# tpfeifle/pointcloud-segmentation-attention

Measured on AMD Instinct MI355X. Metric: 8192-pt clouds/sec through SA+FP layers, 1/2/4/8 MI355X; HBM GB/s vs peak, higher is better.
Workload: dtype f32

## Files before the change

pointcloud-segmentation-attention_amd/csrc/interp.hip:

```cpp
#include <algorithm>
#include <type_traits>

#include "grid.h"

namespace pn2 {
namespace {

constexpr int kNNBlock = 256;
constexpr int kNNGroup = 4;
constexpr int kNNRows = kNNBlock / kNNGroup;
constexpr int kNNTile = 2048;

struct Best3 {
  float d1, d2, d3;
  int i1, i2, i3;
};

PN2_DEV void best3_init(Best3& b) {
  b.d1 = b.d2 = b.d3 = __builtin_inff();
  b.i1 = b.i2 = b.i3 = 0;
}

PN2_DEV void best3_insert(Best3& b, float d, int k) {
  const bool c1 = d < b.d1, c2 = d < b.d2, c3 = d < b.d3;
// ... 86 lines not shown
  best3_merge_xor(best, 2);
}

__global__ __launch_bounds__(kNNBlock) void three_nn_kernel(const float* __restrict__ xyz1,
                                                            const float* __restrict__ xyz2, int n,
                                                            int m, float* __restrict__ dist,
                                                            int32_t* __restrict__ idx) {
  __shared__ float4 sk[kNNTile];
  const int b = blockIdx.y;
  const int j = blockIdx.x * kNNRows + threadIdx.x / kNNGroup;
  const bool valid = j < n;
  const float* U = xyz1 + ((size_t)b * n + (valid ? j : 0)) * 3;
  Best3 best;
  best3_init(best);
  scan_known(xyz2 + (size_t)b * m * 3, m, U[0], U[1], U[2], sk, best);
  if (valid && (threadIdx.x & (kNNGroup - 1)) == 0) {
    float* D = dist + ((size_t)b * n + j) * 3;
    int32_t* I = idx + ((size_t)b * n + j) * 3;
    D[0] = best.d1; D[1] = best.d2; D[2] = best.d3;
    I[0] = best.i1; I[1] = best.i2; I[2] = best.i3;
  }
}


PN2_DEV bool box_certifies(const GridHdr& h, float px, float py, float pz, int xl, int xh,
                           int yl, int yh, int zl, int zh, float d3) {
  if (!(d3 < __builtin_inff())) return false;
  const float edge = 1.0f / h.inv;
  float gap = __builtin_inff();
  auto face = [&](float d, float pc, float o, int c) {
    const float fc = o + (float)c * edge;
    gap = fminf(gap, d - 1e-5f * (fabsf(pc) + fabsf(o) + fabsf(fc) + (float)c * edge) - 1e-30f);
  };
  if (xl > 0) face(px - (h.ox + (float)xl * edge), px, h.ox, xl);
  if (xh < h.nx - 1) face((h.ox + (float)(xh + 1) * edge) - px, px, h.ox, xh + 1);
  if (yl > 0) face(py - (h.oy + (float)yl * edge), py, h.oy, yl);
  if (yh < h.ny - 1) face((h.oy + (float)(yh + 1) * edge) - py, py, h.oy, yh + 1);
  if (zl > 0) face(pz - (h.oz + (float)zl * edge), pz, h.oz, zl);
  if (zh < h.nz - 1) face((h.oz + (float)(zh + 1) * edge) - pz, pz, h.oz, zh + 1);
  return gap > 0.0f && d3 < gap * gap * 0.9999f;
}

PN2_DEV float axis_gap(float p, float o, float edge, int c, int cp) {
  if (c == cp) return 0.0f;
  const int f = c > cp ? c : c + 1;
  const float fc = o + (float)f * edge;
  const float d = c > cp ? fc - p : p - fc;
  return fmaxf(d - 1e-5f * (fabsf(p) + fabsf(o) + fabsf(fc) + (float)f * edge) - 1e-30f, 0.0f);
}
PN2_DEV bool gap_excludes(float g2, float d3) { return d3 < g2 * 0.9999f; }

constexpr int kNNFirst = 1;

template <int G, typename Off>
PN2_DEV Best3 grid_nn3(const GridHdr& h, const float4* __restrict__ pts,
                       const Off* __restrict__ off, float px, float py, float pz, int q) {
  Best3K best;
  best3k_init(best);
  auto merged = [&]() {
    Best3K mb = best;
    if constexpr (G == 4) {
      best3k_merge_quad<kDppXor1>(mb);
      best3k_merge_quad<kDppXor2>(mb);
    }
    return best3_of(mb);
  };
  const int cx = cell_coord(px, h.ox, h.inv, h.nx);
  const int cy = cell_coord(py, h.oy, h.inv, h.ny);
  const int cz = cell_coord(pz, h.oz, h.inv, h.nz);
  Best3 res;
  for (int s = kNNFirst;; ++s) {
    const int xl = cx - s, xh = cx + s, yl = cy - s, yh = cy + s, zl = cz - s, zh = cz + s;
    const int x0 = max(xl, 0), x1 = min(xh, h.nx - 1);
    const bool block = s == kNNFirst;
    auto visit = [&](int lo, int hi) {
      for (int e = lo + q; e < hi; e += G) {
        const float4 p = pts[e];
        best3k_insert(best, nn_key(sqdist(p.x, p.y, p.z, px, py, pz), __float_as_int(p.w)));
      }
    };
    if (block) {
      for (int z = max(zl, 0); z <= min(zh, h.nz - 1); ++z)
        for (int y = max(yl, 0); y <= min(yh, h.ny - 1); ++y) {
          const int row = (z * h.ny + y) * h.nx;
          visit(off[row + x0], off[row + x1 + 1]);
        }
    } else {
      const float d3 = res.d3, edge = 1.0f / h.inv;
#pragma nounroll
      for (int z = max(zl, 0); z <= min(zh, h.nz - 1); ++z) {
        const float gz = axis_gap(pz, h.oz, edge, z, cz), gz2 = gz * gz;
        if (gap_excludes(gz2, d3)) continue;
#pragma nounroll
        for (int y = max(yl, 0); y <= min(yh, h.ny - 1); ++y) {
          const float gy = axis_gap(py, h.oy, edge, y, cy), gyz = gz2 + gy * gy;
          if (gap_excludes(gyz, d3)) continue;
          const int row = (z * h.ny + y) * h.nx;
          const bool face = z == zl || z == zh || y == yl || y == yh;
          int xa = face ? x0 : xl, xb = face ? x1 : xh;
#pragma nounroll
          while (xa <= xb) {
            const float g = axis_gap(px, h.ox, edge, xa, cx);
            if (xa >= 0 && xa < h.nx && !gap_excludes(gyz + g * g, d3)) break;
            xa = face || xa != xl ? xa + 1 : xh;
          }
#pragma nounroll
          while (xb > xa) {
            const float g = axis_gap(px, h.ox, edge, xb, cx);
            if (xb >= 0 && xb < h.nx && !gap_excludes(gyz + g * g, d3)) break;
            xb = face || xb != xh ? xb - 1 : xl;
          }
          if (xa > xb) continue;
          if (face || xa == xb) {
            visit(off[row + xa], off[row + xb + 1]);
          } else {
            visit(off[row + xa], off[row + xa + 1]);
            visit(off[row + xb], off[row + xb + 1]);
          }
        }
      }
    }
    res = merged();
    if (xl <= 0 && yl <= 0 && zl <= 0 && xh >= h.nx - 1 && yh >= h.ny - 1 && zh >= h.nz - 1)
      break;
    if (box_certifies(h, px, py, pz, xl, xh, yl, yh, zl, zh, res.d3)) break;
  }
  return res;
}

template <int G, typename Off>
PN2_DEV Best3 grid_nn3_wave(const GridHdr& h, const float4* __restrict__ pts,
                            const Off* __restrict__ off, float px, float py, float pz, int q,
                            bool valid) {
  if (valid) return grid_nn3<G, Off>(h, pts, off, px, py, pz, q);
  Best3 none;
  best3_init(none);
  return none;
}


template <int BLOCK, bool LDS, int G, int K>
__global__ __launch_bounds__(BLOCK) void three_nn_grid_kernel(
    const void* __restrict__ kgrid, int m, const void* __restrict__ ugrid,
    const float* __restrict__ xyz1, int n, int B, float* __restrict__ dist,
    int32_t* __restrict__ idx) {
  static_assert(G == 1 || G == 4, "one lane or a quad per unknown");
  constexpr int QPB = BLOCK / G;
  extern __shared__ float4 s_pts[];
  const int R = (n + QPB * K - 1) / (QPB * K);
  const int Lg = xcd_block(blockIdx.x, R * B);
// ... 291 lines not shown
#if PN2_FPG_STAMP
__device__ unsigned long long g_fpg_stamp[4096 * 8];
#define PN2_FPG_T(K) if (t == 0 && Lg < 4096) g_fpg_stamp[Lg * 8 + (K)] = __builtin_amdgcn_s_memtime();
#else
#define PN2_FPG_T(K)
#endif

size_t device_lds_per_block() {
  static size_t cache[64] = {0};
  int dev = 0;
  if (hipGetDevice(&dev) != hipSuccess || dev < 0 || dev >= 64) return 64 * 1024;
  if (!cache[dev]) {
    int v = 0, o = 0;
    if (hipDeviceGetAttribute(&v, hipDeviceAttributeMaxSharedMemoryPerBlock, dev) != hipSuccess)
      v = 0;
    if (hipDeviceGetAttribute(&o, hipDeviceAttributeSharedMemPerBlockOptin, dev) != hipSuccess)
      o = 0;
    v = std::max(v, o);
    if (v <= 0) return 64 * 1024;
    cache[dev] = (size_t)v;
  }
  return cache[dev];
}

inline size_t fp_grid_lds(int m) {
  const size_t cells = (size_t)ceil((double)m * kAutoPointsPerCell / kFpgPointsPerCell);
  return (size_t)m * 16 + ((std::max(cells, (size_t)kAutoMinCells) + 1) * 2 + 3) / 4 * 4;
}

template <int V2, int V1, int UN, int KPT, int FB>
__global__ __launch_bounds__(FB) void fp_grid_fused_kernel(FpLayer p, float* __restrict__ dist,
                                                        int32_t* __restrict__ idx,
                                                        const char* __restrict__ kgrid) {
  constexpr int NW = FB / kWave;
  constexpr int FR = FB / kNNGroup;
  extern __shared__ float4 s_pts[];
  __shared__ int4 s_idx[FR];
  __shared__ float s_wv[3][FR];
  float(*red)[NW] = reinterpret_cast<float(*)[NW]>(&s_wv[0][0]);
  int* wsum = reinterpret_cast<int*>(&s_wv[1][0]);
  GridHdr* shp = reinterpret_cast<GridHdr*>(&s_wv[2][0]);
  static_assert(6 * NW <= FR && sizeof(GridHdr) <= FR * 4, "build scratch fits");
  const int n = p.n, m = p.m;
  const int R = (n + FR - 1) / FR;
  const int total = R * p.B;
  const int Lg = xcd_block(blockIdx.x, total);
  if (Lg >= total) return;
  const int b = Lg / R;
  const int j0 = (Lg - b * R) * FR;
  const int t = threadIdx.x, lane = t & (kWave - 1), w = t / kWave;
  uint16_t* s_off = reinterpret_cast<uint16_t*>(s_pts + m);
  uint32_t* s_cnt = reinterpret_cast<uint32_t*>(s_pts + m);
  PN2_FPG_T(0)
  GridHdr h;
  bool built = false;
  if (kgrid) {
    const char* G = kgrid + (size_t)b * grid_stride(m);
    h = *reinterpret_cast<const GridHdr*>(G);
    if (h.ncell >= 1 && h.ncell <= max(m, kAutoMinCells)) {
      const int* goff = reinterpret_cast<const int*>(G + sizeof(GridHdr));
      const float4* gpts = reinterpret_cast<const float4*>(G + kGridOffBytes);
      for (int i = t; i < m; i += FB) s_pts[i] = gpts[i];
      for (int i = t; i <= h.ncell; i += FB) s_off[i] = (uint16_t)goff[i];
      __syncthreads();
      built = true;
    }
  }
  if (!built) {
    const float* __restrict__ K = p.xyz2 + (size_t)b * m * 3;
    float mn[3] = {INFINITY, INFINITY, INFINITY}, mx[3] = {-INFINITY, -INFINITY, -INFINITY};
#pragma unroll
    for (int i = 0; i < KPT; ++i) {
      const int k = t + i * FB;
      if (k < m) {
#pragma unroll
        for (int a = 0; a < 3; ++a) {
          const float v = K[3 * k + a];
          mn[a] = fminf(mn[a], v);
          mx[a] = fmaxf(mx[a], v);
        }
      }
    }
#pragma unroll
    for (int a = 0; a < 3; ++a) {
      mn[a] = wave_min_f(mn[a]);
      mx[a] = wave_max_f(mx[a]);
    }
    if (lane == 0) {
#pragma unroll
      for (int a = 0; a < 3; ++a) { red[a][w] = mn[a]; red[3 + a][w] = mx[a]; }
    }
    __syncthreads();
    if (t == 0) {
      float lo[3], hi[3];
      for (int a = 0; a < 3; ++a) {
        lo[a] = red[a][0];
        hi[a] = red[3 + a][0];
        for (int i = 1; i < NW; ++i) { lo[a] = fminf(lo[a], red[a][i]); hi[a] = fmaxf(hi[a], red[3 + a][i]); }
        if (!(hi[a] >= lo[a])) { lo[a] = 0.0f; hi[a] = 0.0f; }
      }
      *shp = grid_dims(lo, hi, m, 0.0f, kFpgPointsPerCell);
    }
    __syncthreads();
    h = *shp;
    PN2_FPG_T(1)
    auto cell_at = [&](float x, float y, float z) {
      const int ix = cell_coord(x, h.ox, h.inv, h.nx);
      const int iy = cell_coord(y, h.oy, h.inv, h.ny);
      const int iz = cell_coord(z, h.oz, h.inv, h.nz);
      return (iz * h.ny + iy) * h.nx + ix;
    };

    for (int i = t; i < (h.ncell + 2) / 2; i += FB) s_cnt[i] = 0u;
    __syncthreads();
    int kc[KPT], kr[KPT];
#pragma unroll
    for (int i = 0; i < KPT; ++i) {
      const int k = t + i * FB;
      kc[i] = 0;
      kr[i] = 0;
      if (k < m) {
        const int c = cell_at(K[3 * k + 0], K[3 * k + 1], K[3 * k + 2]);
        const int sh = 16 * (c & 1);
        const uint32_t old = atomicAdd(&s_cnt[c >> 1], 1u << sh);
        kc[i] = c;
        kr[i] = (int)((old >> sh) & 0xFFFFu);
      }
    }
    __syncthreads();
    {
      const int per = (h.ncell + FB - 1) / FB;
      const int s0 = t * per, s1 = min(s0 + per, h.ncell);
      int sum = 0;
      for (int i = s0; i < s1; ++i) sum += s_off[i];
      const int incl = wave_incl_scan(sum, lane);
      if (lane == kWave - 1) wsum[w] = incl;
      __syncthreads();
      int base = incl - sum;
      for (int i = 0; i < w; ++i) base += wsum[i];
      for (int i = s0; i < s1; ++i) {
        const int c = s_off[i];
        s_off[i] = (uint16_t)base;
        base += c;
      }
      if (t == 0) s_off[h.ncell] = (uint16_t)m;
    }
    __syncthreads();
#pragma unroll
    for (int i = 0; i < KPT; ++i) {
      const int k = t + i * FB;
      if (k < m)
        s_pts[s_off[kc[i]] + kr[i]] = make_float4(K[3 * k + 0], K[3 * k + 1], K[3 * k + 2],
                                                  __int_as_float(k));
    }
    __syncthreads();
  }

  PN2_FPG_T(2)
  const int jl = t / kNNGroup, q = t & (kNNGroup - 1);
  const int j = j0 + jl;
  {
    const bool valid = j < n;
    const int jc = valid ? j : n - 1;
    float px, py, pz;
    int u;
    if (p.ugrid) {
      const float4 U = grid_view(p.ugrid, b, n).pts[jc];
      px = U.x; py = U.y; pz = U.z;
      u = __float_as_int(U.w);
    } else {
      const float* U = p.xyz1 + ((size_t)b * n + jc) * 3;
      px = U[0]; py = U[1]; pz = U[2];
      u = jc;
    }
    const Best3 res = grid_nn3_wave<kNNGroup, uint16_t>(h, s_pts, s_off, px, py, pz, q, valid);
    if (valid && q == 0) {
      float w1, w2, w3;
      idw(res.d1, res.d2, res.d3, w1, w2, w3);
      s_idx[jl] = make_int4(res.i1, res.i2, res.i3, u);
      s_wv[0][jl] = w1;
      s_wv[1][jl] = w2;
      s_wv[2][jl] = w3;
      if (dist) {
        float* D = dist + ((size_t)b * n + u) * 3;
        int32_t* I = idx + ((size_t)b * n + u) * 3;
        D[0] = res.d1; D[1] = res.d2; D[2] = res.d3;
        I[0] = res.i1; I[1] = res.i2; I[2] = res.i3;
      }
    }
  }
  __syncthreads();
  PN2_FPG_T(3)
  fp_write_rows<V2, V1, UN, FB>(p, b, 0, j0, [&](int rl) {
    const int4 I = s_idx[rl];
    return FpRow{I, make_float4(s_wv[0][rl], s_wv[1][rl], s_wv[2][rl], 0.0f), I.w};
  });
  PN2_FPG_T(4)
}

constexpr int kFpMaxLayers = PN2_FP_MAX_LAYERS;
struct FpLayers {
  FpLayer l[kFpMaxLayers];
  int first[kFpMaxLayers + 1];
  int nlayers, B;
};
template <int V2, int V1, bool PRE, int UN>
__global__ __launch_bounds__(kNNBlock) void fp_fused_layers_kernel(FpLayers a, int tile) {
  extern __shared__ float4 sk[];
  const int per_cloud_all = a.first[a.nlayers];
  const int total = per_cloud_all * a.B;
  const int L = xcd_block(blockIdx.x, total);
  if (L >= total) return;
  const int b = L / per_cloud_all;
  const int lc = L - b * per_cloud_all;
  int li = 0;
  while (li + 1 < a.nlayers && lc >= a.first[li + 1]) ++li;
  const int per_cloud = a.first[li + 1] - a.first[li];
  fp_fused_body<V2, V1, PRE, UN>(a.l[li], b * per_cloud + (lc - a.first[li]), sk, tile);
}

int batch_chunk(int B, int n, int C, int rows) {
  if ((long long)rows * C * C >= (1LL << 32)) return 0;
  long long per_b = (long long)n * n;
  if (per_b >= (1LL << 32)) return 0;
  long long ch = ((1LL << 32) - 1) / (per_b > 0 ? per_b : 1);
  if ((long long)n * ch >= (1LL << 31)) ch = ((1LL << 31) - 1) / (n > 0 ? n : 1);
  return (int)(ch < B ? ch : B);
}

// ... 294 lines not shown
```

pointcloud-segmentation-attention_amd/csrc/fps_cull.h:

```cpp
#pragma once
#include "fps_kernels.h"
#include "grid.h"

namespace pn2 {
namespace {

__device__ unsigned long long g_cull_stats[16 * 8];
__device__ unsigned long long g_cull_wave[16 * 16 * 4];
__device__ unsigned long long g_cull_ev[64 * 16 * 8];

PN2_DEV int wave_max_i32_l63(int v) {
#define PN2_IMAX_DPP(C, R) v = max(v, __builtin_amdgcn_update_dpp(0, v, C, R, 0xF, false))
  PN2_IMAX_DPP(kDppXor1, 0xF);
  PN2_IMAX_DPP(kDppXor2, 0xF);
  PN2_IMAX_DPP(kDppHalfMirror, 0xF);
  PN2_IMAX_DPP(kDppMirror, 0xF);
#undef PN2_IMAX_DPP
  asm volatile(
      "s_nop 1\n\t"
      "v_max_i32_dpp %0, %0, %0 row_bcast:15 row_mask:0xa bank_mask:0xf\n\t"
      "s_nop 1\n\t"
      "v_max_i32_dpp %0, %0, %0 row_bcast:31 row_mask:0xc bank_mask:0xf\n\t"
      "s_nop 1"
      : "+v"(v));
  return v;
}

PN2_DEV uint32_t cull_key(int k) { return ((uint32_t)(k & 511) << 16) | ((uint32_t)k >> 9); }

PN2_DEV uint32_t point_hash(uint32_t x, uint32_t y, uint32_t z) {
  uint32_t h = x ^ __builtin_rotateleft32(y, 11) ^ __builtin_rotateleft32(z, 22);
  h = (h ^ (h >> 16)) * 0x85EBCA6Bu;
  h = (h ^ (h >> 13)) * 0xC2B2AE35u;
  return h ^ (h >> 16);
}
#ifndef PN2_FPS_DEDUP_ROUNDS
#define PN2_FPS_DEDUP_ROUNDS 2
#endif
constexpr int kDedupRounds = PN2_FPS_DEDUP_ROUNDS;

__device__ unsigned long long g_cull_dedup[16 * 4];

PN2_DEV uint32_t wave_excl_scan(uint32_t v, int lane) {
  uint32_t s = v;
#pragma unroll
  for (int o = 1; o < kWave; o <<= 1) {
    const uint32_t u = (uint32_t)__shfl_up((int)s, o, kWave);
    s += lane >= o ? u : 0u;
  }
  return s - v;
}

PN2_DEV float box_lb(float4 lo, float4 hi, float cx, float cy, float cz) {
  const float gx = fmaxf(fmaxf(lo.x - cx, cx - hi.x), 0.0f);
  const float gy = fmaxf(fmaxf(lo.y - cy, cy - hi.y), 0.0f);
  const float gz = fmaxf(fmaxf(lo.z - cz, cz - hi.z), 0.0f);
  return (gx * gx + gy * gy) + gz * gz;
}

__constant__ float kCullFrac[12] = {0.6f, 0.7f, 0.75f, 0.8f, 0.84f, 0.87f,
                                    0.9f, 0.92f, 0.94f, 0.96f, 0.98f, 0.99f};


#define PN2_EV(K)                                                                          \
  if constexpr (STAMP) ev[K] = __builtin_amdgcn_s_memtime();

template <int PPT, int GRP>
PN2_DEV constexpr uint64_t cell_lanes(int s) {
  uint64_t m = 0;
  for (int i = 0; i < GRP; ++i) m |= 1ull << (PPT * i + s);
  return m;
}

using hf2 = float __attribute__((ext_vector_type(2)));

PN2_DEV void hot_best4(const int (&hv)[4], const hf2 (&hx)[2], const hf2 (&hy)[2],
           const hf2 (&hz)[2], const int (&hk)[4], int& cv, float& lx, float& ly,
           float& lz, int& lk, int& wm, uint64_t& m01, uint64_t& m23, uint64_t& mh) {
  int v23, r, tk;
  float tx, ty, tz;
  asm volatile(
      "v_cmp_gt_i32_e64 %[m01], %[h1], %[h0]\n\t"
      "v_cmp_gt_i32_e64 %[m23], %[h3], %[h2]\n\t"
      "v_max_i32_e32 %[cv], %[h0], %[h1]\n\t"
      "v_max_i32_e32 %[v23], %[h2], %[h3]\n\t"
      "v_cmp_gt_i32_e64 %[mh], %[v23], %[cv]\n\t"
      "v_max_i32_e32 %[cv], %[cv], %[v23]\n\t"
      "v_cndmask_b32_e64 %[lx], %[x0], %[x1], %[m01]\n\t"
      "v_cndmask_b32_e64 %[tx], %[x2], %[x3], %[m23]\n\t"
      "v_max_i32_dpp %[r], %[cv], %[cv] quad_perm:[1,0,3,2] row_mask:0xf bank_mask:0xf\n\t"
      "v_cndmask_b32_e64 %[ly], %[y0], %[y1], %[m01]\n\t"
      "v_cndmask_b32_e64 %[ty], %[y2], %[y3], %[m23]\n\t"
// ... 378 lines not shown
    for (int c = 0; c < NCW; ++c)
      if ((c + 1) % 4 == 0) m |= 1u << c;
    return m;
  }();
  constexpr int kWantD = PPC == 1 ? 2 : 1;
#endif
  constexpr int kSpare = NCELL - (NPTS + CP - 1) / CP;
  constexpr int kNLW = __builtin_popcount(kLight);
  constexpr int kPerW = kSpare / (kNLW > 0 ? kNLW : 1);
  constexpr int kLD = kNLW == 0 ? 0 : (kPerW < kWantD ? kPerW : kWantD);
  constexpr int kNL = kLD > 0 ? __builtin_popcount(kLight) : 0;
  static_assert(kLight < (1u << NCW), "light waves are cold waves");
  static_assert((NCELL - kNL * kLD) * CP >= NPTS, "light layout capacity");
  const int lbefore = cw >= 0 ? __builtin_popcount(kLight & ((1u << cw) - 1u)) : 0;
  const bool light = cw >= 0 && ((kLight >> cw) & 1u);
  auto cellof = [&](int s) {
    if (kNL == 0 || s < PPT - kLD) return s * NCW + cw;
    const int q = s - (PPT - kLD);
    if (!light) return s * NCW - kNL * q + cw - lbefore;
    return NCELL - kNL * kLD + q * kNL + lbefore;
  };
  auto spos = [&](int s, int h) { return cellof(s) * CP + h * kWave + lane; };
#define PN2_CELLMAX(s) wave_max_i32(PPC == 1 ? tb[(s) * PPC] : max(tb[(s) * PPC], tb[(s) * PPC + PPC - 1]))
  int Tm[PPT];
  float4 glo = make_float4(INFINITY, INFINITY, INFINITY, 0.0f), ghi = make_float4(-INFINITY, -INFINITY, -INFINITY, 0.0f);
  int tmv = -1;
  if (cw >= 0) {
#pragma unroll
    for (int s = 0; s < PPT; ++s) {
      bool any = false;
#pragma unroll
      for (int h = 0; h < PPC; ++h) {
        const int pos = spos(s, h);
        const bool in = pos < Np;
        const int k = in ? sperm[pos] : 0;
        px[s * PPC + h] = X[3 * k];
        py[s * PPC + h] = X[3 * k + 1];
        if constexpr (ZLDS) scz[(cw * PPT * PPC + s * PPC + h) * kWave + lane] = X[3 * k + 2];
        else pz[s * PPC + h] = X[3 * k + 2];
        tb[s * PPC + h] = in ? __float_as_int(kInitTemp) : -1;
        any = any || __builtin_amdgcn_ballot_w64(in) != 0;
      }
      Tm[s] = any ? __float_as_int(kInitTemp) : -1;
    }
    if (lane < GRP * PPT) {
      glo = scell[2 * cellof(lane % PPT)];
      ghi = scell[2 * cellof(lane % PPT) + 1];
    }
#pragma unroll
    for (int s = 0; s < PPT; ++s) tmv = lane % PPT == s ? Tm[s] : tmv;
  }
  PN2_STAMP(7)

  int j = 0;
  int rp = 0;
  int tlo = 2;
  int T = 0, nh = 0;
  bool hot_turn = false;
  uint32_t dirty = 0;
  auto round_end = [&](auto cold_tag, int round) -> bool {
    constexpr bool COLD = decltype(cold_tag)::value;
    __syncthreads();
    PN2_EV(2)
    PN2_STAMP(2)
    j += sj[rp] & (kEnd - 1);
    if (j >= M) return true;
    if constexpr (STAMP) ++n_refresh;
    int top;
    {
      const int v = lane < NW ? swmax[lane] : -1;
      top = __builtin_amdgcn_readfirstlane(wave_max_i32(v));
    }
    int tau[NWIN];
    {
      const float tf = __int_as_float(max(top, 0));
#pragma unroll
      for (int i = 0; i < NWIN; ++i)
        tau[i] = (int)uniform_u32((uint32_t)__float_as_int(tf * kCullFrac[tlo + i]));
    }
    if constexpr (COLD) {
      uint32_t c0 = 0, c1 = 0, c2 = 0, c3 = 0;
      static_assert(NWIN == 4, "four counters");
#pragma unroll
      for (int s = 0; s < PPT; ++s) {
        if (Tm[s] > tau[0]) {
#pragma unroll
          for (int h = 0; h < PPC; ++h) {
            const int e = s * PPC + h;
            c0 += __builtin_popcountll(__builtin_amdgcn_ballot_w64(tb[e] > tau[0]));
            c1 += __builtin_popcountll(__builtin_amdgcn_ballot_w64(tb[e] > tau[1]));
            c2 += __builtin_popcountll(__builtin_amdgcn_ballot_w64(tb[e] > tau[2]));
            c3 += __builtin_popcountll(__builtin_amdgcn_ballot_w64(tb[e] > tau[3]));
          }
        }
      }
      if (lane < NWIN) swcnt[w][lane] = lane == 0 ? c0 : lane == 1 ? c1 : lane == 2 ? c2 : c3;
    }
    PN2_EV(3)
    PN2_STAMP(3)
    __syncthreads();
    PN2_EV(4)
    PN2_STAMP(4)
    const int cvw = lane & 15, ciw = lane >> 4;
    const uint32_t cnt = cvw < NW ? swcnt[cvw][ciw] : 0u;
    uint32_t tot = cnt;
#define PN2_ADD_DPP(C) tot += (uint32_t)__builtin_amdgcn_update_dpp(0, (int)tot, C, 0xF, 0xF, false)
    PN2_ADD_DPP(kDppXor1);
    PN2_ADD_DPP(kDppXor2);
    PN2_ADD_DPP(kDppHalfMirror);
    PN2_ADD_DPP(kDppMirror);
#undef PN2_ADD_DPP
    const uint64_t fit = __builtin_amdgcn_ballot_w64(cvw == 0 && tot >= 1u && tot <= (uint32_t)K);
    const int ti = fit ? (int)__builtin_ctzll(fit) >> 4 : -1;
    const bool stall = ti < 0;
    T = 0;
#pragma unroll
    for (int i = 0; i < NWIN; ++i) T = ti == i ? tau[i] : T;
    nh = stall ? 0 : __builtin_amdgcn_readlane((int)tot, ti * 16);
// ... 39 lines not shown
    } else {
      uint64_t best = 0;
      if constexpr (COLD) {
#pragma unroll
        for (int e = 0; e < PPT * PPC; ++e) {
          const uint64_t v = tb[e] < 0 ? 0ull
                                       : pack64(~cull_key(sperm[spos(e / PPC, e % PPC)]),
                                                (uint32_t)tb[e] + 1u);
          best = v > best ? v : best;
        }
        best = wave_max_u64(best);
      }
      if (lane == 0) swk[w] = best;
      if constexpr (STAMP) ++n_stall;
    }
    PN2_EV(5)
    PN2_STAMP(5)
    __syncthreads();
    PN2_EV(6)
    PN2_STAMP(6)
    if constexpr (STAMP) {
      if (b == 0 && lane == 0 && round < 64) {
#pragma unroll
        for (int k = 0; k < 8; ++k) g_cull_ev[(round * 16 + w) * 8 + k] = ev[k];
      }
    }
    if (stall) {
      uint64_t best = lane < NW ? swk[lane] : 0ull;
      best = uniform_u64(wave_max_u64(best));
      const uint32_t key = ~(uint32_t)best;
      const int k = (int)((key >> 16) + ((key & 0xFFFFu) << 9));
      if (top <= 0) {
        for (int e = j + t; e < M; e += BLOCK) {
          I[e] = k;
          if (NX) {
            NX[3 * e] = X[3 * k];
            NX[3 * e + 1] = X[3 * k + 1];
            NX[3 * e + 2] = X[3 * k + 2];
          }
        }
        return true;
      }
      if (t == 0) {
        scl[0] = make_float4(X[3 * k], X[3 * k + 1], X[3 * k + 2],
                             __uint_as_float((uint32_t)k | pick_tag(j)));
        publish_end(&sj[rp ^ 1], 1 | kEnd);
      }
    }
    hot_turn = !stall;
    rp ^= 1;
    PN2_STAMP(6)
    return false;
  };
  if (w == 0) {
    for (int round = 0; round <= M; ++round) {
      if (hot_turn) {
        static_assert(HQ == 2 || HQ == 4, "hot entries per lane");
        int hv[HQ], hk[HQ];
        uint32_t hkey[HQ];
        float qx[HQ], qy[HQ], qz[HQ];
#pragma unroll
        for (int q = 0; q < HQ; ++q) {
          const int e = lane + q * kWave;
          if constexpr (LEAN) {
            const uint4 en = e < nh ? shx[e] : make_uint4(0xFFFFFFFFu, 0u, 0u, 0u);
            qz[q] = e < nh ? shz[e] : 0.0f;
            hv[q] = (int)en.x;
            hk[q] = (int)en.y;
            qx[q] = __uint_as_float(en.z);
            qy[q] = __uint_as_float(en.w);
          } else {
            const uint2 en = e < nh ? sh[e] : make_uint2(0xFFFFFFFFu, 0u);
            hv[q] = (int)en.x;
            hk[q] = (int)en.y;
          }
          hkey[q] = hv[q] >= 0 ? cull_key(hk[q]) : 0xFFFFFFFFu;
        }
#pragma unroll
        for (int pass = 0; pass < HQ; ++pass) {
#pragma unroll
          for (int q = pass & 1; q + 1 < HQ; q += 2) {
            if (hkey[q + 1] < hkey[q]) {
              const int v = hv[q], k = hk[q];
              const uint32_t y = hkey[q];
              hv[q] = hv[q + 1]; hk[q] = hk[q + 1]; hkey[q] = hkey[q + 1];
              hv[q + 1] = v; hk[q + 1] = k; hkey[q + 1] = y;
              if constexpr (LEAN) {
                const float ax = qx[q], ay = qy[q], az = qz[q];
                qx[q] = qx[q + 1]; qy[q] = qy[q + 1]; qz[q] = qz[q + 1];
                qx[q + 1] = ax; qy[q + 1] = ay; qz[q + 1] = az;
              }
            }
          }
        }
        constexpr int HP = HQ / 2;
        f2 hx[HP], hy[HP], hz[HP];
#pragma unroll
        for (int q = 0; q < HQ; ++q) {
          hx[q / 2][q % 2] = LEAN ? qx[q] : X[3 * hk[q]];
          hy[q / 2][q % 2] = LEAN ? qy[q] : X[3 * hk[q] + 1];
          hz[q / 2][q % 2] = LEAN ? qz[q] : X[3 * hk[q] + 2];
          hk[q] |= (int)pick_tag(j);
        }
        const int lim = min(K, M - j);
        int jj = 0;
        if constexpr (PRIO > 0) __builtin_amdgcn_s_setprio(PRIO);
        __builtin_amdgcn_s_waitcnt(0xC07F);
// ... 16 lines not shown
              cv = b01 ? hv[1] : hv[0];
              lx = b01 ? hx[0][1] : hx[0][0];
              ly = b01 ? hy[0][1] : hy[0][0];
              lz = b01 ? hz[0][1] : hz[0][0];
              lk = b01 ? hk[1] : hk[0];
              asm volatile("" ::"v"(lx), "v"(ly), "v"(lz), "v"(lk));
              wm = __builtin_amdgcn_readlane(wave_max_i32_l63(cv), 63);
            }
            if (!(wm > T)) break;
            const uint64_t hold = __builtin_amdgcn_ballot_w64(cv == wm);
            int L;
            if (__builtin_popcountll(hold) == 1) {
              L = (int)__builtin_ctzll(hold);
            } else {
              if constexpr (STAMP) ++n_tie;
              uint32_t ck;
              if constexpr (HQ == 4) {
                uint32_t k23;
                asm volatile("v_cndmask_b32_e64 %0, %1, %2, %3" : "=v"(ck)
                             : "v"(hkey[0]), "v"(hkey[1]), "s"(m01));
                asm volatile("v_cndmask_b32_e64 %0, %1, %2, %3" : "=v"(k23)
                             : "v"(hkey[2]), "v"(hkey[3]), "s"(m23));
                asm volatile("v_cndmask_b32_e64 %0, %0, %1, %2" : "+v"(ck) : "v"(k23), "s"(mh));
              } else {
                ck = hv[1] > hv[0] ? hkey[1] : hkey[0];
              }
              const uint32_t km = ~uniform_u32(wave_max_u32(cv == wm ? ~ck : 0u));
              L = (int)__builtin_ctzll(__builtin_amdgcn_ballot_w64(cv == wm && ck == km));
            }
            float cx, cy, cz;
            hot_publish(L, va_c, va_n, vcnt, lx, ly, lz, lk, cx, cy, cz);
            __builtin_amdgcn_sched_barrier(0);
            hot_update<HP>(hv, hx, hy, hz, cx, cy, cz);
            va_c += 16;
            vcnt += 1;
            if constexpr (CHECKED)
              if (__builtin_amdgcn_readfirstlane(vcnt) >= lim) break;
          }
        };
        if (lim >= K) pick_loop(std::false_type{});
        else if (lim > 0) pick_loop(std::true_type{});
        jj = __builtin_amdgcn_readfirstlane(vcnt);
        if constexpr (PRIO > 0) __builtin_amdgcn_s_setprio(0);
        if (lane == 0) publish_end(&sj[rp], jj | kEnd);
        if constexpr (STAMP) {
          n_hot += jj;
        }
      }
      PN2_EV(0)
      PN2_STAMP(7)
      if (round_end(std::false_type{}, round)) break;
    }
  } else {
    for (int round = 0; round <= M; ++round) {
      int applied = 0;
      bool stop = false;
      unsigned long long tcnt0 = 0;
      int it = 0;
      for (; it < PN2_FPS_POLL_LIMIT; ++it) {
        const int sv = __builtin_amdgcn_readfirstlane(
            __hip_atomic_load(&sj[rp], __ATOMIC_ACQUIRE, __HIP_MEMORY_SCOPE_WORKGROUP));
        const int av = sv & (kEnd - 1);
        stop = (sv & kEnd) != 0;
        if (av - applied >= GRP || (stop && av > applied)) {
          const int a1 = min(av, applied + GRP);
          const int ci = applied + lane / PPT;
          const bool valid = lane < GRP * PPT && ci < a1;
          const float4 cv = scl[valid ? ci : 0];
          if (__builtin_amdgcn_ballot_w64(
                  valid && (__float_as_uint(cv.w) & ~kPickIdxMask) != pick_tag(j))) {
            PN2_TORN_SEEN();
            continue;
          }
          if constexpr (PRIO > 0) __builtin_amdgcn_s_setprio(PRIO - 1);
          if constexpr (STAMP) tcnt0 = __builtin_amdgcn_s_memtime();
          if (cw == 0 && valid && lane % PPT == 0) {
            I[j + ci] = (int)(__float_as_uint(cv.w) & kPickIdxMask);
            if (NX) {
              NX[3 * (j + ci)] = cv.x;
              NX[3 * (j + ci) + 1] = cv.y;
              NX[3 * (j + ci) + 2] = cv.z;
            }
          }
          const float lb = box_lb(glo, ghi, cv.x, cv.y, cv.z);
          const uint64_t m = __builtin_amdgcn_ballot_w64(valid && __float_as_int(lb) < tmv);
          if constexpr (STAMP) n_pairs += __builtin_popcountll(m);
          if (m) {
#pragma unroll
            for (int s = 0; s < PPT; ++s) {
              uint64_t ms = m & cell_lanes<PPT, GRP>(s);
              if (!ms) continue;
              while (ms) {
                const int la = (int)__builtin_ctzll(ms);
                ms &= ms - 1;
                const int lb2 = ms ? (int)__builtin_ctzll(ms) : la;
                ms &= ms ? ms - 1 : 0;
                const float ax = __builtin_bit_cast(float, __builtin_amdgcn_readlane(__float_as_int(cv.x), la));
                const float ay = __builtin_bit_cast(float, __builtin_amdgcn_readlane(__float_as_int(cv.y), la));
                const float az = __builtin_bit_cast(float, __builtin_amdgcn_readlane(__float_as_int(cv.z), la));
                const float bx = __builtin_bit_cast(float, __builtin_amdgcn_readlane(__float_as_int(cv.x), lb2));
                const float by = __builtin_bit_cast(float, __builtin_amdgcn_readlane(__float_as_int(cv.y), lb2));
                const float bz = __builtin_bit_cast(float, __builtin_amdgcn_readlane(__float_as_int(cv.z), lb2));
                const f2 cx = {ax, bx}, cy = {ay, by}, cz = {az, bz};
#pragma unroll
                for (int h = 0; h < PPC; ++h) {
                  const int e = s * PPC + h;
                  const float zz = ZLDS ? scz[(cw * PPT * PPC + e) * kWave + lane] : pz[e];
                  const f2 qx = {px[e], px[e]}, qy = {py[e], py[e]}, qz = {zz, zz};
                  const f2 dx = qx - cx, dy = qy - cy, dz = qz - cz;
                  const f2 d = (dx * dx + dy * dy) + dz * dz;
                  tb[e] = min(min(tb[e], __float_as_int(d.x)), __float_as_int(d.y));
                }
              }
              dirty |= 1u << s;
            }
          }
          applied = a1;
          if constexpr (PRIO > 0) __builtin_amdgcn_s_setprio(0);
          if constexpr (STAMP) {
            n_tail_grp += stop ? 1 : 0;
            const unsigned long long dt = __builtin_amdgcn_s_memtime() - tcnt0;
            n_grp += 1;
            n_grp_cyc += dt;
          }
          continue;
        }
        if (stop) break;
        if (dirty) {
          const int s0 = __builtin_ctz(dirty);
#pragma unroll
          for (int s = 0; s < PPT; ++s) {
            if (s == s0) {
              Tm[s] = __builtin_amdgcn_readfirstlane(PN2_CELLMAX(s));
              tmv = lane % PPT == s ? Tm[s] : tmv;
            }
          }
          dirty &= dirty - 1;
          continue;
        }
        if constexpr (STAMP) ++n_poll;
      }
      if (it == PN2_FPS_POLL_LIMIT && fault && lane == 0)
        __hip_atomic_store(fault, PN2_FAULT_FPS_POLL, __ATOMIC_RELAXED, __HIP_MEMORY_SCOPE_SYSTEM);
      PN2_EV(0)
      PN2_STAMP(0)
      int wmax = -1;
#pragma unroll
      for (int s = 0; s < PPT; ++s)
        if (!(dirty & (1u << s))) wmax = max(wmax, Tm[s]);
#pragma unroll
      for (int s = 0; s < PPT; ++s) {
        if ((dirty & (1u << s)) && Tm[s] > wmax) {
          Tm[s] = __builtin_amdgcn_readfirstlane(PN2_CELLMAX(s));
          tmv = lane % PPT == s ? Tm[s] : tmv;
          dirty &= ~(1u << s);
          wmax = max(wmax, Tm[s]);
        }
      }
      if (lane == 0) swmax[w] = wmax;
      PN2_EV(1)
      PN2_STAMP(1)
      if (round_end(std::true_type{}, round)) break;
    }
  }
  if constexpr (KG) {
    __syncthreads();
    if (char* const G = s_kgrid) {
      __shared__ GridHdr sgh;
      block_grid_build<BLOCK>(NX, M, G, shist, sbox, swmax, &sgh, w * kWave + (int)__lane_id());
    }
  }
  if constexpr (STAMP) {
    if (lane == 0 && b < 16) {
#pragma unroll
      for (int ph = 0; ph < 8; ++ph) g_stamp[(b * 16 + w) * 8 + ph] = st_acc[ph];
      g_cull_wave[(b * 16 + w) * 4 + 0] = n_grp;
      g_cull_wave[(b * 16 + w) * 4 + 1] = n_grp_cyc;
      g_cull_wave[(b * 16 + w) * 4 + 2] = n_pairs;
      g_cull_wave[(b * 16 + w) * 4 + 3] = n_poll;
      if (w == 0) {
        g_cull_stats[b * 8 + 0] = __builtin_amdgcn_s_memtime() - clk0;
        g_cull_stats[b * 8 + 1] = n_refresh;
        g_cull_stats[b * 8 + 2] = n_stall;
        g_cull_stats[b * 8 + 4] = n_hot;
        g_cull_dedup[b * 4 + 0] = (unsigned long long)Np;
        g_cull_dedup[b * 4 + 1] = dd_clk;
        g_cull_dedup[b * 4 + 2] = n_tie;
      }
      if (w == 1) {
        g_cull_stats[b * 8 + 3] = n_pairs;
        g_cull_stats[b * 8 + 7] = n_tail_grp;
      }
      if (w == 2) g_cull_stats[b * 8 + 5] = n_pairs;
    }
  }
}

template <int NW, int PPT, int NPTS, bool STAMP = false, int PRIO = 0, int HQ = 2, int PPC = 1,
          bool LEAN = false>
__global__ __launch_bounds__(64 * NW) void fps_hotcull_kernel(const float* __restrict__ xyz, int N,
                                                           int M, int32_t* __restrict__ idx,
                                                           float* __restrict__ new_xyz,
                                                           int* __restrict__ fault) {
  hotcull_body<NW, PPT, NPTS, STAMP, PRIO, HQ, PPC, LEAN>(xyz, N, M, idx, new_xyz, fault);
}

template <int NW, int PPT, int NPTS, int PRIO, int HQ>
__global__ __launch_bounds__(64 * NW) void fps_hotcull_grid_kernel(const float* __restrict__ xyz,
                                                                int N, int M,
                                                                int32_t* __restrict__ idx,
                                                                float* __restrict__ new_xyz,
                                                                int* __restrict__ fault,
                                                                char* __restrict__ kgrid) {
  hotcull_body<NW, PPT, NPTS, false, PRIO, HQ, 1, false, true>(xyz, N, M, idx, new_xyz, fault,
                                                               kgrid);
}

template <int NW, int PPT, int PRIO = 0, int HQ = 2, int NPTS = 8192, int PPC = 1,
          bool LEAN = false>
void launch_hotcull(const float* xyz, int B, int N, int M, int32_t* idx, float* nx, int* fault,
                    hipStream_t s) {
  hipLaunchKernelGGL((fps_hotcull_kernel<NW, PPT, NPTS, false, PRIO, HQ, PPC, LEAN>), dim3(B),
                     dim3(64 * NW), 0, s, xyz, N, M, idx, nx, fault);
}

template <int NW, int PPT, int PRIO = 0, int HQ = 2, int NPTS = 8192>
void launch_hotcull_grid(const float* xyz, int B, int N, int M, int32_t* idx, float* nx,
                         int* fault, hipStream_t s, char* kgrid) {
  hipLaunchKernelGGL((fps_hotcull_grid_kernel<NW, PPT, NPTS, PRIO, HQ>), dim3(B), dim3(64 * NW),
                     0, s, xyz, N, M, idx, nx, fault, kgrid);
}

}
}
```

Before: 102,900.

## Stage only the z-slab of grid cells the block's queries need into LDS

Before staging the prebuilt grid, each block computes the z-cell range covered by its query rows and copies only the points and offsets for that slab (padded by one ring) into shared memory. The search runs on the slab copy and falls back to a global-memory search over the full grid whenever it would need to expand beyond the slab. This cuts the per-block global read and LDS fill of the full key cloud, at the cost of a wave reduction, a possibly divergent slower fallback path, and swapping the wave-level search helper for the generic one.

Result: no change. 102,400 (-0.5%).

```diff
diff --git a/pointcloud-segmentation-attention_amd/csrc/interp.hip b/pointcloud-segmentation-attention_amd/csrc/interp.hip
--- a/pointcloud-segmentation-attention_amd/csrc/interp.hip
+++ b/pointcloud-segmentation-attention_amd/csrc/interp.hip
@@ -162,9 +162,10 @@
 
 constexpr int kNNFirst = 1;
 
-template <int G, typename Off>
+template <int G, typename Off, bool SLAB = false>
 PN2_DEV Best3 grid_nn3(const GridHdr& h, const float4* __restrict__ pts,
-                       const Off* __restrict__ off, float px, float py, float pz, int q) {
+                       const Off* __restrict__ off, float px, float py, float pz, int q,
+                       int cbase = 0, int zs0 = 0, int zs1 = 0, bool* left = nullptr) {
   Best3K best;
   best3k_init(best);
   auto merged = [&]() {
@@ -183,6 +184,13 @@
     const int xl = cx - s, xh = cx + s, yl = cy - s, yh = cy + s, zl = cz - s, zh = cz + s;
     const int x0 = max(xl, 0), x1 = min(xh, h.nx - 1);
     const bool block = s == kNNFirst;
+    if constexpr (SLAB) {
+      if (!block && (max(zl, 0) < zs0 || min(zh, h.nz - 1) > zs1)) {
+        *left = true;
+        best3_init(res);
+        return res;
+      }
+    }
     auto visit = [&](int lo, int hi) {
       for (int e = lo + q; e < hi; e += G) {
         const float4 p = pts[e];
@@ -192,7 +200,7 @@
     if (block) {
       for (int z = max(zl, 0); z <= min(zh, h.nz - 1); ++z)
         for (int y = max(yl, 0); y <= min(yh, h.ny - 1); ++y) {
-          const int row = (z * h.ny + y) * h.nx;
+          const int row = (z * h.ny + y) * h.nx - cbase;
           visit(off[row + x0], off[row + x1 + 1]);
         }
     } else {
@@ -205,7 +213,7 @@
         for (int y = max(yl, 0); y <= min(yh, h.ny - 1); ++y) {
           const float gy = axis_gap(py, h.oy, edge, y, cy), gyz = gz2 + gy * gy;
           if (gap_excludes(gyz, d3)) continue;
-          const int row = (z * h.ny + y) * h.nx;
+          const int row = (z * h.ny + y) * h.nx - cbase;
           const bool face = z == zl || z == zh || y == yl || y == yh;
           int xa = face ? x0 : xl, xb = face ? x1 : xh;
 #pragma nounroll
@@ -603,16 +611,50 @@
   uint16_t* s_off = reinterpret_cast<uint16_t*>(s_pts + m);
   uint32_t* s_cnt = reinterpret_cast<uint32_t*>(s_pts + m);
   PN2_FPG_T(0)
+  const int jl = t / kNNGroup, q = t & (kNNGroup - 1);
+  const bool valid = j0 + jl < n;
+  float px, py, pz;
+  int u;
+  {
+    const int jc = valid ? j0 + jl : n - 1;
+    if (p.ugrid) {
+      const float4 U = grid_view(p.ugrid, b, n).pts[jc];
+      px = U.x; py = U.y; pz = U.z;
+      u = __float_as_int(U.w);
+    } else {
+      const float* U = p.xyz1 + ((size_t)b * n + jc) * 3;
+      px = U[0]; py = U[1]; pz = U[2];
+      u = jc;
+    }
+  }
   GridHdr h;
   bool built = false;
+  int cbase = 0, zs0 = 0, zs1 = 0;
+  const int* goff = nullptr;
+  const float4* gpts = nullptr;
   if (kgrid) {
     const char* G = kgrid + (size_t)b * grid_stride(m);
     h = *reinterpret_cast<const GridHdr*>(G);
     if (h.ncell >= 1 && h.ncell <= max(m, kAutoMinCells)) {
-      const int* goff = reinterpret_cast<const int*>(G + sizeof(GridHdr));
-      const float4* gpts = reinterpret_cast<const float4*>(G + kGridOffBytes);
-      for (int i = t; i < m; i += FB) s_pts[i] = gpts[i];
-      for (int i = t; i <= h.ncell; i += FB) s_off[i] = (uint16_t)goff[i];
+      goff = reinterpret_cast<const int*>(G + sizeof(GridHdr));
+      gpts = reinterpret_cast<const float4*>(G + kGridOffBytes);
+      static_assert(FR == kWave, "a lane of every wave per row");
+      const int jz = min(j0 + lane, n - 1);
+      const float rz = p.ugrid ? grid_view(p.ugrid, b, n).pts[jz].z
+                               : p.xyz1[((size_t)b * n + jz) * 3 + 2];
+      const int cz = cell_coord(rz, h.oz, h.inv, h.nz);
+      const int lo = dpp_reduce<kWave>(cz, [](int a, int c) { return min(a, c); });
+      zs0 = max((int)uniform_u32(lo) - kNNFirst, 0);
+      zs1 = min((int)uniform_u32(wave_max_i32(cz)) + kNNFirst, h.nz - 1);
+      cbase = zs0 * h.ny * h.nx;
+      const int cells = (zs1 - zs0 + 1) * h.ny * h.nx;
+      const int p0 = min(max(goff[cbase], 0), m);
+      const int np = min(max(goff[cbase + cells], p0), m) - p0;
+      for (int i = t; i < np; i += FB) s_pts[i] = gpts[p0 + i];
+      for (int i = t; i <= cells; i += FB) s_off[i] = (uint16_t)(goff[cbase + i] - p0);
+#if PN2_FPG_STAMP
+      if (t == 0 && Lg < 4096) { g_fpg_stamp[Lg * 8 + 5] = np; g_fpg_stamp[Lg * 8 + 6] = 0; }
+#endif
       __syncthreads();
       built = true;
     }
@@ -705,27 +747,21 @@
                                                   __int_as_float(k));
     }
     __syncthreads();
+    zs1 = h.nz - 1;
   }
 
   PN2_FPG_T(2)
-  const int jl = t / kNNGroup, q = t & (kNNGroup - 1);
-  const int j = j0 + jl;
-  {
-    const bool valid = j < n;
-    const int jc = valid ? j : n - 1;
-    float px, py, pz;
-    int u;
-    if (p.ugrid) {
-      const float4 U = grid_view(p.ugrid, b, n).pts[jc];
-      px = U.x; py = U.y; pz = U.z;
-      u = __float_as_int(U.w);
-    } else {
-      const float* U = p.xyz1 + ((size_t)b * n + jc) * 3;
-      px = U[0]; py = U[1]; pz = U[2];
-      u = jc;
-    }
-    const Best3 res = grid_nn3_wave<kNNGroup, uint16_t>(h, s_pts, s_off, px, py, pz, q, valid);
-    if (valid && q == 0) {
+  if (valid) {
+    bool left = false;
+    Best3 res = grid_nn3<kNNGroup, uint16_t, true>(h, s_pts, s_off, px, py, pz, q, cbase, zs0,
+                                                   zs1, &left);
+    if (left) {
+      res = grid_nn3<kNNGroup, int>(h, gpts, goff, px, py, pz, q);
+#if PN2_FPG_STAMP
+      if (q == 0 && Lg < 4096) atomicAdd(&g_fpg_stamp[Lg * 8 + 6], 1ull);
+#endif
+    }
+    if (q == 0) {
       float w1, w2, w3;
       idw(res.d1, res.d2, res.d3, w1, w2, w3);
       s_idx[jl] = make_int4(res.i1, res.i2, res.i3, u);
```

## Run first FPS picks as lockstep brute-force rounds before hot/cold cull protocol

Applied to the files above, without the earlier changes.

Adds an early phase in which every wave brute-force updates its owned point distances and reduces a block-wide argmax through double-buffered shared slots and one barrier per pick. It does this for the first few picks (default 16, or 8 in the message layout) before entering the hot/cold culling pipeline. While the distance bounds are still loose, culling saves little and the polling handshake costs a lot, and this phase is meant to replace it. It also hides the lane-to-cell modulo behind an opaque asm so it is not recomputed in the dirty-refresh loop. The trade-off is more shared state and a more complex tie-break path that has to match the original pick order.

New measurement: 102,500 before, 103,500 after (median of 5 runs). +1.0%, better.

```diff
diff --git a/pointcloud-segmentation-attention_amd/csrc/fps_cull.h b/pointcloud-segmentation-attention_amd/csrc/fps_cull.h
--- a/pointcloud-segmentation-attention_amd/csrc/fps_cull.h
+++ b/pointcloud-segmentation-attention_amd/csrc/fps_cull.h
@@ -38,6 +38,12 @@
 #define PN2_FPS_DEDUP_ROUNDS 2
 #endif
 constexpr int kDedupRounds = PN2_FPS_DEDUP_ROUNDS;
+#ifndef PN2_FPS_EARLY_PICKS
+#define PN2_FPS_EARLY_PICKS 16
+#endif
+#ifndef PN2_FPS_EARLY_PICKS_MSG
+#define PN2_FPS_EARLY_PICKS_MSG 8
+#endif
 
 __device__ unsigned long long g_cull_dedup[16 * 4];
 
@@ -522,6 +528,11 @@
   }
   PN2_STAMP(7)
 
+  auto cell_of_lane = [&] {
+    int l = lane;
+    asm volatile("" : "+v"(l));
+    return l % PPT;
+  };
   int j = 0;
   int rp = 0;
   int tlo = 2;
@@ -534,6 +545,7 @@
     PN2_EV(2)
     PN2_STAMP(2)
     j += sj[rp] & (kEnd - 1);
+    if constexpr (STAMP) ev[7] = (unsigned long long)(sj[rp] & (kEnd - 1));
     if (j >= M) return true;
     if constexpr (STAMP) ++n_refresh;
     int top;
@@ -679,7 +691,136 @@
     PN2_STAMP(6)
     return false;
   };
+  constexpr int kEarly = PPC == 2 ? PN2_FPS_EARLY_PICKS_MSG : PN2_FPS_EARLY_PICKS;
+  __shared__ uint64_t sek[2][NW];
+  __shared__ float4 sec[2][NW];
+  unsigned long long early_clk = 0;
+  auto early = [&](auto cold_tag) -> bool {
+    constexpr bool COLD = decltype(cold_tag)::value;
+    constexpr int NE = PPT * PPC;
+    const int E = min(kEarly, M - 1);
+    if (kEarly <= 0 || E <= 0) return false;
+    if constexpr (STAMP) early_clk = __builtin_amdgcn_s_memtime();
+    auto uni = [](float v) {
+      return __builtin_bit_cast(float, __builtin_amdgcn_readfirstlane(__float_as_int(v)));
+    };
+    float4 c = make_float4(uni(X[0]), uni(X[1]), uni(X[2]), __int_as_float(0));
+    static_assert(kEarly <= K, "the early picks wait in the batch slots");
+    auto flush = [&](int n) {
+      for (int x = lane; x < n; x += kWave) {
+        const float4 pk = scl[x];
+        I[x] = __float_as_int(pk.w);
+        if (NX) {
+          NX[3 * x] = pk.x;
+          NX[3 * x + 1] = pk.y;
+          NX[3 * x + 2] = pk.z;
+        }
+      }
+    };
+    uint32_t occ0 = 0;
+    if constexpr (COLD) {
+#pragma unroll
+      for (int s = 0; s < PPT; ++s) occ0 |= Tm[s] >= 0 ? 1u << s : 0u;
+    }
+    for (int e = 1; e <= E; ++e) {
+      const int buf = e & 1;
+      if constexpr (COLD) {
+        uint32_t occ = occ0;
+        asm volatile("" : "+s"(occ));
+        const f2 c2x = {c.x, c.x}, c2y = {c.y, c.y}, c2z = {c.z, c.z};
+        auto zof = [&](int i) { return ZLDS ? scz[(cw * NE + i) * kWave + lane] : pz[i]; };
+        int lv = -1;
+#pragma unroll
+        for (int i = 0; i < NE; i += 2) {
+          const int i1 = i + 1 < NE ? i + 1 : i;
+          if (!(occ & (1u << (i / PPC) | 1u << (i1 / PPC)))) continue;
+          const f2 qx = {px[i], px[i1]}, qy = {py[i], py[i1]}, qz = {zof(i), zof(i1)};
+          const f2 dx = qx - c2x, dy = qy - c2y, dz = qz - c2z;
+          const f2 d = (dx * dx + dy * dy) + dz * dz;
+          tb[i] = min(tb[i], __float_as_int(d.x));
+          tb[i1] = min(tb[i1], __float_as_int(d.y));
+          lv = max(lv, max(tb[i], tb[i1]));
+        }
+        const int wm = __builtin_amdgcn_readfirstlane(wave_max_i32(lv));
+        uint32_t bk = 0xFFFFFFFFu;
+        float bx = 0.0f, by = 0.0f, bz = 0.0f;
+        if (wm >= 0) {
+#pragma unroll
+          for (int i = 0; i < NE; ++i) {
+            if (!(occ & 1u << (i / PPC))) continue;
+            if (__builtin_amdgcn_ballot_w64(tb[i] == wm) == 0) continue;
+            if (tb[i] == wm) {
+              const uint32_t key = cull_key(sperm[spos(i / PPC, i % PPC)]);
+              if (key < bk) {
+                bk = key;
+                bx = px[i];
+                by = py[i];
+                bz = zof(i);
+              }
+            }
+          }
+        }
+        if (wm < 0) {
+          if (lane == 0) sek[buf][w] = 0ull;
+        } else {
+          const uint64_t hold = __builtin_amdgcn_ballot_w64(bk != 0xFFFFFFFFu);
+          const uint32_t km =
+              __builtin_popcountll(hold) == 1
+                  ? (uint32_t)__builtin_amdgcn_readlane((int)bk, (int)__builtin_ctzll(hold))
+                  : ~uniform_u32(wave_max_u32(~bk));
+          if (bk == km) {
+            const int k = (int)((km >> 16) + ((km & 0xFFFFu) << 9));
+            sek[buf][w] = pack64(~km, (uint32_t)wm + 1u);
+            sec[buf][w] = make_float4(bx, by, bz, __int_as_float(k));
+          }
+        }
+      } else {
+        if (lane == 0) {
+          sek[buf][w] = 0ull;
+          scl[e - 1] = c;
+        }
+      }
+      __syncthreads();
+      const uint64_t mine = lane < NW ? sek[buf][lane] : 0ull;
+      const float4 mc = sec[buf][lane < NW ? lane : 0];
+      const uint64_t best = uniform_u64(row16_max_u64(mine));
+      if ((uint32_t)(best >> 32) <= 1u) {
+        const uint32_t key = ~(uint32_t)best;
+        const int k = min((int)((key >> 16) + ((key & 0xFFFFu) << 9)), N - 1);
+        if constexpr (!COLD) flush(e);
+        for (int x = e + w * kWave + lane; x < M; x += BLOCK) {
+          I[x] = k;
+          if (NX) {
+            NX[3 * x] = X[3 * k];
+            NX[3 * x + 1] = X[3 * k + 1];
+            NX[3 * x + 2] = X[3 * k + 2];
+          }
+        }
+        return true;
+      }
+      const int wv = (int)__builtin_ctzll(__builtin_amdgcn_ballot_w64(lane < NW && mine == best));
+      auto from = [&](float v) {
+        return __builtin_bit_cast(float, __builtin_amdgcn_readlane(__float_as_int(v), wv));
+      };
+      c = make_float4(from(mc.x), from(mc.y), from(mc.z), from(mc.w));
+    }
+    if constexpr (COLD) {
+      dirty = occ0;
+    } else {
+      flush(E);
+      if (lane == 0) {
+        scl[0] = make_float4(c.x, c.y, c.z, __uint_as_float(__float_as_uint(c.w) | pick_tag(E)));
+        sj[0] = 1 | kEnd;
+      }
+      if constexpr (STAMP) early_clk = __builtin_amdgcn_s_memtime() - early_clk;
+    }
+    j = E;
+    __syncthreads();
+    PN2_STAMP(7)
+    return false;
+  };
   if (w == 0) {
+    if (early(std::false_type{})) goto sampled;
     for (int round = 0; round <= M; ++round) {
       if (hot_turn) {
         static_assert(HQ == 2 || HQ == 4, "hot entries per lane");
@@ -802,6 +943,7 @@
       if (round_end(std::false_type{}, round)) break;
     }
   } else {
+    if (early(std::true_type{})) goto sampled;
     for (int round = 0; round <= M; ++round) {
       int applied = 0;
       bool stop = false;
@@ -878,11 +1020,12 @@
         if (stop) break;
         if (dirty) {
           const int s0 = __builtin_ctz(dirty);
+          const int lcell = cell_of_lane();
 #pragma unroll
           for (int s = 0; s < PPT; ++s) {
             if (s == s0) {
               Tm[s] = __builtin_amdgcn_readfirstlane(PN2_CELLMAX(s));
-              tmv = lane % PPT == s ? Tm[s] : tmv;
+              tmv = lcell == s ? Tm[s] : tmv;
             }
           }
           dirty &= dirty - 1;
@@ -902,7 +1045,7 @@
       for (int s = 0; s < PPT; ++s) {
         if ((dirty & (1u << s)) && Tm[s] > wmax) {
           Tm[s] = __builtin_amdgcn_readfirstlane(PN2_CELLMAX(s));
-          tmv = lane % PPT == s ? Tm[s] : tmv;
+          tmv = cell_of_lane() == s ? Tm[s] : tmv;
           dirty &= ~(1u << s);
           wmax = max(wmax, Tm[s]);
         }
@@ -913,6 +1056,7 @@
       if (round_end(std::true_type{}, round)) break;
     }
   }
+sampled:
   if constexpr (KG) {
     __syncthreads();
     if (char* const G = s_kgrid) {
@@ -936,6 +1080,8 @@
         g_cull_dedup[b * 4 + 0] = (unsigned long long)Np;
         g_cull_dedup[b * 4 + 1] = dd_clk;
         g_cull_dedup[b * 4 + 2] = n_tie;
+        g_cull_dedup[b * 4 + 3] =
+            early_clk | (unsigned long long)max(min(kEarly, M - 1), 0) << 48;
       }
       if (w == 1) {
         g_cull_stats[b * 8 + 3] = n_pairs;
```
